# 0xC0000054/pdn-jpegxl

Measured on AMD Instinct MI355X. Metric: megapixels/sec decode (4K lossy VarDCT), higher is better.
Workload: dtype f32

## Files before the change

pdn_jpegxl_amd/build.py:

```python
import os
import subprocess
import sys

HERE = os.path.dirname(os.path.abspath(__file__))
CSRC = os.path.join(HERE, "csrc")
LIBDIR = os.path.join(HERE, "lib")
LIBNAME = "libJpegXLFileTypeIO_X64.so"
TEST_LIBNAME = "libjxlhip_selftest.so"
TEST_SOURCES = ["selftest.cc"]
SOURCES = ["kernels.hip", "entropy_kernels.hip", "tile_kernels.hip", "encode_kernels.hip", "lossless_kernels.hip", "distance_kernels.hip", "compose_kernels.hip", "patch_kernels.hip", "noise_kernels.hip", "downscale_kernels.hip", "host_parse.cc", "host_write.cc", "icc.cc", "decoder.cc", "encoder.cc"]
HEADERS = ["dev_types.h", "dev_util.h", "modular_uniform.h", "enc_types.h", "enc_dev.h", "kernels.h", "host_parse.h", "host_write.h", "icc.h", os.path.join("..", "..", "include", "jxlfiletypeio.h")]


def lib_path():
    return os.path.join(LIBDIR, LIBNAME)


def test_lib_path():
    return os.path.join(LIBDIR, TEST_LIBNAME)


def source_digest():
    import hashlib
    h = hashlib.sha256()
    for name in SOURCES + TEST_SOURCES + HEADERS:
        with open(os.path.join(CSRC, name), "rb") as f:
            h.update(name.encode() + b"\0" + f.read() + b"\0")
    return h.hexdigest()


def manifest_text(extra=None):
    if extra is None:
        extra = os.environ.get("JXLHIP_EXTRA_CFLAGS", "")
    extra = " ".join(extra.split())
    return source_digest() + ("\nextra: " + extra if extra else "") + "\n"


def manifest_path():
    return os.path.join(LIBDIR, "sources.sha256")


def _stale(out, deps):
    if not os.path.exists(out):
        return True
# ... 64 lines not shown
```

pdn_jpegxl_amd/csrc/entropy_kernels.hip:

```cpp
#include <hip/hip_runtime.h>
#include <cstdlib>
#include "dev_types.h"
#include "dev_util.h"
#include "kernels.h"

namespace jxlhip {

namespace {

__device__ const uint8_t d_order_bucket[kNumStrategies] = {0, 1, 1, 1, 2, 3, 4, 4, 5, 5, 6, 6, 1, 1, 1, 1, 1, 1, 7, 8, 8, 9, 10, 10, 11, 12, 12};
__device__ const uint8_t d_log2cx[kNumStrategies] = {0, 0, 0, 0, 1, 2, 0, 1, 0, 2, 1, 2, 0, 0, 0, 0, 0, 0, 3, 2, 3, 4, 3, 4, 5, 4, 5};
__device__ const uint8_t d_log2cy[kNumStrategies] = {0, 0, 0, 0, 1, 2, 1, 0, 2, 0, 2, 1, 0, 0, 0, 0, 0, 0, 3, 3, 2, 4, 4, 3, 5, 5, 4};
__device__ const uint8_t d_nnz_ctx[64] = {0,   0,   31,  62,  62,  93,  93,  93,  93,  123, 123, 123, 123, 152, 152, 152, 152, 152, 152, 152, 152, 180,
                                          180, 180, 180, 180, 180, 180, 180, 180, 180, 180, 180, 206, 206, 206, 206, 206, 206, 206, 206, 206, 206, 206,
                                          206, 206, 206, 206, 206, 206, 206, 206, 206, 206, 206, 206, 206, 206, 206, 206, 206, 206, 206, 206};

__device__ __forceinline__ int CeilLog2D(uint32_t x) { return x <= 1 ? 0 : 32 - __clz(x - 1); }
__device__ __forceinline__ int32_t UnpackSigned(uint32_t u) { return (int32_t)(u >> 1) ^ -(int32_t)(u & 1); }
#ifndef JXLHIP_PRIO_SERIAL
#define JXLHIP_PRIO_SERIAL 0
#endif
#if JXLHIP_PRIO_SERIAL
#define JXL_SERIAL_PRIO() __builtin_amdgcn_s_setprio(JXLHIP_PRIO_SERIAL)
#else
#define JXL_SERIAL_PRIO() ((void)0)
#endif

__device__ __forceinline__ void SetError(const DevImage& im, uint32_t bits, int who = 0, int where = 0) {
  atomicOr(im.status, bits);
  if (who) im.status[2 + who] = (uint32_t)where + 1;
}

#define JXL_LDS __attribute__((address_space(3)))
#define JXL_GLB __attribute__((address_space(1)))
template <class T> __device__ __forceinline__ JXL_GLB T* G(T* p) { return (JXL_GLB T*)p; }
typedef int __attribute__((ext_vector_type(4))) I4;
typedef unsigned __attribute__((ext_vector_type(2))) U2;
typedef unsigned __attribute__((ext_vector_type(4))) U4;

constexpr int kRingWords = 32;
constexpr int kTopUpEvery = 16;
template <int kRing, int kBatch>
struct LaneBitsT {
  const JXL_GLB uint32_t* w;
  JXL_LDS uint32_t* ring;
  uint32_t rs;
  uint32_t nwords;
  uint32_t rd, filled;
  uint64_t buf;
  int n;
  int skip;
  uint32_t pend[kBatch];
  bool has_pend;
  JXL_GLB uint32_t* lz_win;
  uint32_t lz_mask, lz_dm, lz_copy, lz_src, lz_done, slow_err;
  __device__ __forceinline__ void SetLz(uint32_t* win, uint32_t log_size, uint32_t dist_mult) {
    lz_win = (JXL_GLB uint32_t*)win; lz_mask = (1u << log_size) - 1; lz_dm = dist_mult;
  }
  __device__ __forceinline__ void Fetch(uint32_t* v) {
    static_assert(kBatch == 4 || kBatch == 8, "one or two 16-byte loads");
    if (filled + kBatch <= nwords) {
      const U4 a = *(const JXL_GLB U4*)(w + filled);
      v[0] = a.x; v[1] = a.y; v[2] = a.z; v[3] = a.w;
      if constexpr (kBatch == 8) {
        const U4 c = *(const JXL_GLB U4*)(w + filled + 4);
        v[4] = c.x; v[5] = c.y; v[6] = c.z; v[7] = c.w;
      }
    } else {
#pragma unroll
      for (int i = 0; i < kBatch; i++) v[i] = filled + i < nwords ? w[filled + i] : 0u;
    }
  }
  __device__ __forceinline__ void Stage(const uint32_t* v) {
#pragma unroll
    for (int i = 0; i < kBatch; i++) ring[__umul24((filled + i) & (kRing - 1), rs)] = v[i];
    filled += kBatch;
  }
  __device__ __forceinline__ void Batch() {
    uint32_t v[kBatch];
    Fetch(v);
    Stage(v);
  }
  __device__ __forceinline__ void TopUpSync() {
    while (filled + kBatch <= rd + kRing) Batch();
  }
  __device__ __forceinline__ void TopUp() {
    if (has_pend) { Stage(pend); has_pend = false; }
    while (filled + kBatch <= rd + kRing && filled - rd < (uint32_t)(kRing * 3 / 4)) Batch();
    if (filled + kBatch <= rd + kRing) { Fetch(pend); has_pend = true; }
  }
  __device__ __forceinline__ void Init(const uint8_t* cs, uint64_t cs_size, uint64_t bit_off, JXL_LDS uint32_t* ring_slot, uint32_t ring_stride) {
    const uintptr_t addr = (uintptr_t)cs + (bit_off >> 3);
    const uintptr_t al = addr & ~(uintptr_t)31;
    w = (const JXL_GLB uint32_t*)al;
    ring = ring_slot; rs = ring_stride;
    const uintptr_t end = ((uintptr_t)cs + cs_size + 3) & ~(uintptr_t)3;
    nwords = end > al ? (uint32_t)((end - al) >> 2) : 0u;
    rd = 0; filled = 0; buf = 0; n = 0; has_pend = false;
    lz_win = nullptr; lz_mask = 0; lz_dm = 0; lz_copy = 0; lz_src = 0; lz_done = 0; slow_err = 0;
    skip = (int)(addr - al) * 8 + (int)(bit_off & 7);
    TopUpSync();
    rd = (uint32_t)skip >> 5;
    Refill();
    const int s2 = skip & 31;
    buf >>= s2;
    n -= s2;
  }
  __device__ __forceinline__ void Refill() {
    if (n <= 32) {
      buf |= (uint64_t)ring[__umul24(rd & (kRing - 1), rs)] << n;
      n += 32;
      rd++;
    }
  }
  __device__ __forceinline__ uint32_t Read(int k) {
    Refill();
    const uint32_t v = (uint32_t)(buf & (((uint64_t)1 << k) - 1));
    buf >>= k;
    n -= k;
    return v;
  }
  __device__ uint64_t Consumed() const { return (uint64_t)rd * 32 - n - skip; }
};
typedef LaneBitsT<kRingWords, 8> LaneBits;

template <bool kLds> struct AS;
template <> struct AS<true> {
  typedef const JXL_LDS uint8_t* U8;
  typedef const JXL_LDS uint16_t* U16;
  typedef const JXL_LDS uint32_t* U32;
  typedef const JXL_LDS uint64_t* U64;
  typedef const JXL_LDS I4* Tree;
  typedef JXL_LDS int32_t* Row;
};
template <> struct AS<false> {
  typedef const uint8_t* U8;
  typedef const uint16_t* U16;
  typedef const uint32_t* U32;
  typedef const uint64_t* U64;
  typedef const I4* Tree;
  typedef int32_t* Row;
};

template <bool kLds>
struct CodeTab {
  typename AS<kLds>::U8 cmap;
  typename AS<kLds>::U32 cfg;
  typename AS<kLds>::U64 alias;
  const uint32_t* direct;
  uint32_t log_alpha;
  uint32_t slow;
  const DevCode* dc;
};

__device__ __forceinline__ DevTreeNode NodeOf(I4 v) {
  DevTreeNode n;
  n.property = v.x; n.splitval = v.y; n.a = (uint32_t)v.z; n.b = (uint32_t)v.w;
  return n;
}

template <class Bits>
__device__ __forceinline__ uint32_t HybridTail(Bits& b, uint32_t c, uint32_t sym) {
  const uint32_t se = c & 0xF, split = 1u << se;
  if (sym < split) return sym;
  const uint32_t msb = (c >> 4) & 0xF, lsb = (c >> 8) & 0xF;
  const uint32_t nb = se - (msb + lsb) + ((sym - split) >> (msb + lsb));
  const uint32_t low = sym & ((1u << lsb) - 1);
  const uint32_t t = sym >> lsb;
  const uint32_t bits = b.Read(nb > 32 ? 32 : nb);
  const uint32_t hi = (1u << msb) | (t & ((1u << msb) - 1));
  return (uint32_t)(((((uint64_t)hi << nb) | bits) << lsb) | low);
}

template <bool kLds>
__device__ __forceinline__ uint32_t AnsSym(LaneBits& b, uint32_t& state, typename AS<kLds>::U64 abase, uint32_t log_alpha) {
  const uint32_t le = 12 - log_alpha;
  const uint32_t res = state & 0xFFF, i = res >> le, pos = res & ((1u << le) - 1);
  const uint64_t e = abase[i];
  const uint32_t x = (uint32_t)e, y = (uint32_t)(e >> 32);
  const bool g = pos >= (x & 0xFF);
  const uint32_t sym = g ? ((x >> 8) & 0xFF) : i;
  const uint32_t off = g ? (y & 0xFFFF) + pos : pos;
  const uint32_t freq = g ? ((x >> 16) ^ (y >> 16)) : (x >> 16);
  state = __umul24(freq, state >> 12) + off;
  if (state < 65536u) state = (state << 16) | b.Read(16);
  return sym;
}

template <bool kLds>
__device__ __forceinline__ uint64_t AnsPrefetch(uint32_t state, typename AS<kLds>::U64 abase, uint32_t log_alpha) {
  return abase[(state & 0xFFF) >> (12 - log_alpha)];
}
template <bool kLds>
__device__ __forceinline__ uint32_t AnsSymPf(LaneBits& b, uint32_t& state, typename AS<kLds>::U64 abase, uint32_t log_alpha, uint64_t& e) {
  const uint32_t le = 12 - log_alpha;
  const uint32_t res = state & 0xFFF, i = res >> le, pos = res & ((1u << le) - 1);
  const uint32_t x = (uint32_t)e, y = (uint32_t)(e >> 32);
  const bool g = pos >= (x & 0xFF);
  const uint32_t sym = g ? ((x >> 8) & 0xFF) : i;
  const uint32_t off = g ? (y & 0xFFFF) + pos : pos;
  const uint32_t freq = g ? ((x >> 16) ^ (y >> 16)) : (x >> 16);
  state = __umul24(freq, state >> 12) + off;
  if (state < 65536u) state = (state << 16) | b.Read(16);
  e = abase[(state & 0xFFF) >> le];
  return sym;
}

__device__ const int8_t d_special_dist[120][2] = {
    {0, 1}, {1, 0}, {1, 1}, {-1, 1}, {0, 2}, {2, 0}, {1, 2}, {-1, 2}, {2, 1}, {-2, 1}, {2, 2}, {-2, 2}, {0, 3}, {3, 0}, {1, 3},
    {-1, 3}, {3, 1}, {-3, 1}, {2, 3}, {-2, 3}, {3, 2}, {-3, 2}, {0, 4}, {4, 0}, {1, 4}, {-1, 4}, {4, 1}, {-4, 1}, {3, 3}, {-3, 3},
    {2, 4}, {-2, 4}, {4, 2}, {-4, 2}, {0, 5}, {3, 4}, {-3, 4}, {4, 3}, {-4, 3}, {5, 0}, {1, 5}, {-1, 5}, {5, 1}, {-5, 1}, {2, 5},
    {-2, 5}, {5, 2}, {-5, 2}, {4, 4}, {-4, 4}, {3, 5}, {-3, 5}, {5, 3}, {-5, 3}, {0, 6}, {6, 0}, {1, 6}, {-1, 6}, {6, 1}, {-6, 1},
    {2, 6}, {-2, 6}, {6, 2}, {-6, 2}, {4, 5}, {-4, 5}, {5, 4}, {-5, 4}, {3, 6}, {-3, 6}, {6, 3}, {-6, 3}, {0, 7}, {7, 0}, {1, 7},
    {-1, 7}, {5, 5}, {-5, 5}, {7, 1}, {-7, 1}, {4, 6}, {-4, 6}, {6, 4}, {-6, 4}, {2, 7}, {-2, 7}, {7, 2}, {-7, 2}, {3, 7}, {-3, 7},
    {7, 3}, {-7, 3}, {5, 6}, {-5, 6}, {6, 5}, {-6, 5}, {8, 0}, {4, 7}, {-4, 7}, {7, 4}, {-7, 4}, {8, 1}, {8, 2}, {6, 6}, {-6, 6},
    {8, 3}, {5, 7}, {-5, 7}, {7, 5}, {-7, 5}, {8, 4}, {6, 7}, {-6, 7}, {7, 6}, {-7, 6}, {8, 5}, {7, 7}, {-7, 7}, {8, 6}, {8, 7}};

template <bool kLds, class Bits>
__device__ __forceinline__ uint32_t SlowSymbol(Bits& b, uint32_t& state, const CodeTab<kLds>& t, uint32_t cl) {
  const DevCode& dc = *t.dc;
  if (dc.slow & 1) {
    const uint32_t c = t.cfg[cl];
    if (c & 0x1000) return c >> 16;
    b.Refill();
    const uint32_t bits = (uint32_t)b.buf;
    const uint16_t* cnt = dc.pfx_count + cl * 16;
    int code = 0, first = 0, index = 0;
    for (int l = 1; l < 16; l++) {
      code |= (bits >> (l - 1)) & 1;
      const int k = cnt[l];
      if (code - k < first) {
        b.buf >>= l; b.n -= l;
        return dc.pfx_sorted[dc.pfx_off[cl] + index + code - first];
      }
      index += k; first = (first + k) << 1; code <<= 1;
    }
    b.slow_err = 1;
// ... 35 lines not shown
    dist = min(dist, min(b.lz_done, 1u << 20));
    if (dist == 0 || b.lz_done > b.lz_mask + 1) { b.slow_err = 1; return 0; }
    b.lz_src = b.lz_done - dist;
    b.lz_copy = len - 1;
    const uint32_t v = b.lz_win[(b.lz_src++) & b.lz_mask];
    b.lz_win[(b.lz_done++) & b.lz_mask] = v;
    return v;
  }
  const uint32_t v = HybridTail(b, t.cfg[cl], sym);
  if (lz) b.lz_win[(b.lz_done++) & b.lz_mask] = v;
  return v;
}
template <bool kLds, class Bits>
__device__ __forceinline__ uint32_t InitAnsState(Bits& b, const CodeTab<kLds>& t) { return (t.slow & 1) ? 0x130000u : b.Read(32); }

template <bool kLds, class Bits>
__device__ __forceinline__ uint32_t AnsGet(Bits& b, uint32_t& state, const CodeTab<kLds>& t, uint32_t ctx) {
  if (t.slow) return SlowGet(b, state, t, ctx);
  const uint32_t cl = t.cmap[ctx];
  const uint32_t le = 12 - t.log_alpha;
  const uint32_t res = state & 0xFFF, i = res >> le, pos = res & ((1u << le) - 1);
  const uint64_t e = t.alias[(cl << t.log_alpha) | i];
  const uint32_t c = t.cfg[cl];
  const uint32_t x = (uint32_t)e, y = (uint32_t)(e >> 32);
  const bool g = pos >= (x & 0xFF);
  const uint32_t sym = g ? ((x >> 8) & 0xFF) : i;
  const uint32_t off = g ? (y & 0xFFFF) + pos : pos;
  const uint32_t freq = g ? ((x >> 16) ^ (y >> 16)) : (x >> 16);
  state = __umul24(freq, state >> 12) + off;
  if (state < 65536u) state = (state << 16) | b.Read(16);
  return HybridTail(b, c, sym);
}

__device__ __forceinline__ size_t StageCode(JXL_LDS uint8_t* smem, size_t off, const DevCode& dc, CodeTab<true>& t, int tid, int nt,
                                            bool one_section = false) {
  const uint32_t na = (dc.slow & 1) ? 0u : dc.num_clusters << dc.log_alpha;
  t.direct = (one_section && !dc.slow) ? dc.direct : nullptr;
  off = (off + 7) & ~(size_t)7;
  JXL_LDS uint64_t* sa = (JXL_LDS uint64_t*)(smem + off); off += (size_t)na * 8;
  JXL_LDS uint32_t* sc = (JXL_LDS uint32_t*)(smem + off); off += (size_t)dc.num_clusters * 4;
  JXL_LDS uint8_t* sm = smem + off; off += dc.num_ctx;
  for (uint32_t i = tid; i < na; i += nt) sa[i] = dc.alias[i];
  for (uint32_t i = tid; i < dc.num_clusters; i += nt) sc[i] = dc.cfg[i];
  for (uint32_t i = tid; i < dc.num_ctx; i += nt) sm[i] = dc.ctx_map[i];
  t.cmap = sm; t.cfg = sc; t.alias = sa; t.log_alpha = dc.log_alpha; t.slow = dc.slow; t.dc = &dc;
  return off;
}

__device__ __forceinline__ void GlobalCode(const DevCode& dc, CodeTab<false>& t) {
  t.cmap = dc.ctx_map; t.cfg = dc.cfg; t.alias = dc.alias; t.direct = nullptr; t.log_alpha = dc.log_alpha; t.slow = dc.slow; t.dc = &dc;
}

template <bool kLds>
struct RowBuf {
  typename AS<kLds>::Row rb;
  int rb_stride;
  int rb_width;
};

template <bool kLds, int kPred>
__device__ __forceinline__ void LeafRow(LaneBits& b, uint32_t& state, const CodeTab<kLds>& tab, const DevTreeNode& leaf, int w, int y,
                                        JXL_GLB int32_t* row, int stride, typename AS<kLds>::Row rb, int rs, bool use_rb) {
  const uint32_t cl = tab.cmap[leaf.a >> 8];
  const uint32_t cfg = tab.cfg[cl];
  const typename AS<kLds>::U64 abase = tab.alias + (cl << tab.log_alpha);
  const bool constant_token = (cfg & 0x1000) && ((cfg >> 16) & 0xFF) < (1u << (cfg & 0xF));
  const uint32_t const_res = (uint32_t)UnpackSigned((cfg >> 16) & 0xFF) * leaf.b + (uint32_t)leaf.splitval;
  const JXL_GLB int32_t* prow = row - stride;
  int32_t W = y ? (use_rb ? rb[0] : prow[0]) : 0, N = W, NW = W;
  uint64_t entry = constant_token ? 0 : AnsPrefetch<kLds>(state, abase, tab.log_alpha);
  for (int x = 0; x < w; x++) {
    if ((x & (kTopUpEvery - 1)) == 0) b.TopUp();
    int32_t NE = N;
    if (kPred != 0 && kPred != 1) {
      if (x + 1 < w && y) NE = use_rb ? rb[(x + 1) * rs] : prow[x + 1];
    }
    uint32_t guess;
    if (kPred == 0) guess = 0;
    else if (kPred == 1) guess = (uint32_t)W;
    else if (kPred == 2) guess = (uint32_t)N;
    else {
      const int64_t mn = W < N ? W : N, mx = W < N ? N : W, gr = (int64_t)W + N - NW;
      guess = (uint32_t)(int32_t)(gr < mn ? mn : (gr > mx ? mx : gr));
    }
    uint32_t res;
    if (constant_token) res = const_res;
    else {
      const uint32_t sym = AnsSymPf<kLds>(b, state, abase, tab.log_alpha, entry);
      res = (uint32_t)UnpackSigned(HybridTail(b, cfg, sym)) * leaf.b + (uint32_t)leaf.splitval;
    }
    const int32_t val = (int32_t)(res + guess);
    row[x] = val;
    if (use_rb) rb[x * rs] = val;
    W = val;
    if (y) { NW = N; N = NE; } else { NW = val; N = val; }
  }
}

struct WpState {
  int32_t* err;
  uint32_t* pe;
  int w2;
  int64_t prediction[4];
  int64_t pred;
  __device__ void Init(int32_t* scratch, int w) {
    w2 = w + 2;
    err = scratch;
    pe = (uint32_t*)(err + 2 * w2);
    for (int i = 0; i < 10 * w2; i++) err[i] = 0;
  }
  static __device__ __forceinline__ uint32_t Div(uint32_t i) { return (1u << 24) / (i + 1); }
  static __device__ __forceinline__ uint32_t ErrorWeight(uint64_t x, uint32_t maxweight) {
    int shift = (63 - __clzll((long long)(x + 1))) - 5;
    if (shift < 0) shift = 0;
    return 4 + (uint32_t)((maxweight * (uint64_t)Div((uint32_t)(x >> shift))) >> shift);
  }
  static __device__ __forceinline__ int64_t Abs(int64_t v) { return v < 0 ? -v : v; }
  __device__ int64_t Predict(int x, int y, int w, int64_t N, int64_t W, int64_t NE, int64_t NW, int64_t NN, int64_t* max_err) {
    const int cur = (y & 1) ? 0 : w2, prev = (y & 1) ? w2 : 0;
    const int pN = prev + x, pNE = x < w - 1 ? pN + 1 : pN, pNW = x > 0 ? pN - 1 : pN;
    const uint32_t kW[4] = {13, 12, 12, 12};
    uint32_t weights[4];
// ... 327 lines not shown
    const uint32_t cl = tab.cmap[nd.a >> 8];
    const uint32_t cfg = tab.cfg[cl];
    const typename AS<kLds>::U64 abase = tab.alias + (cl << tab.log_alpha);
    const uint32_t mul = nd.b, off = (uint32_t)nd.splitval;
    const bool add_w = !needs_n && (nd.a & 0xFF) == 1;
    const uint32_t csym = (cfg >> 16) & 0xFF;
    const bool ctok = (cfg & 0x1000) && csym < (1u << (cfg & 0xF));
    const uint32_t cres = (uint32_t)UnpackSigned(csym) * mul + off;
    JXL_GLB int32_t* const row = out + (size_t)y * stride;
    uint32_t W = y ? first_prev : 0u;
    if (ctok) {
      for (int x = 0; x < w; x++) {
        const uint32_t val = cres + (add_w ? W : 0u);
        row[x] = (int32_t)val;
        W = val;
      }
      first_prev = cres + (add_w ? (y ? first_prev : 0u) : 0u);
      continue;
    }
    uint32_t first = 0;
    if constexpr (kLds) {
      if (tab.direct) {
        const uint64_t ga = (uint64_t)(uintptr_t)(tab.direct + (cl << 12));
        const ConstU32 dt = (ConstU32)(((uint64_t)(uint32_t)__builtin_amdgcn_readfirstlane((int)(ga >> 32)) << 32) |
                                       (uint32_t)__builtin_amdgcn_readfirstlane((int)(uint32_t)ga));
        if (mul == 1 && off == 0 && needs_n) RowScalar<true, ConstU32>(b, state, dt, cfg, 1u, 0u, false, W, first, row, w);
        else RowScalar<false, ConstU32>(b, state, dt, cfg, mul, off, add_w, W, first, row, w);
        first_prev = first;
        continue;
      }
    }
    uint64_t entry = AnsPrefetch<kLds>(state, abase, tab.log_alpha);
    for (int x0 = 0; x0 < w; x0 += kTopUpEvery) {
      b.TopUp();
      const int xe = min(w, x0 + kTopUpEvery);
      for (int x = x0; x < xe; x++) {
        const uint32_t sym = AnsSymPf<kLds>(b, state, abase, tab.log_alpha, entry);
        const uint32_t val = (uint32_t)UnpackSigned(HybridTail(b, cfg, sym)) * mul + off + (add_w ? W : 0u);
        row[x] = (int32_t)val;
        W = val;
        first = x == 0 ? val : first;
      }
    }
    first_prev = first;
  }
  d.kind = needs_n ? kChanResid : kChanFinal;
  *desc = d;
}

__device__ __forceinline__ int32_t FromLaneBelow(int32_t v) {
  return __builtin_amdgcn_update_dpp(0, v, 0x138 , 0xF, 0xF, false);
}
__device__ __forceinline__ int32_t ClampedGradient32(int32_t W, int32_t N, int32_t NW) {
  const int32_t mn = W < N ? W : N, mx = W < N ? N : W;
  return NW >= mx ? mn : (NW <= mn ? mx : (int32_t)((uint32_t)W + (uint32_t)N - (uint32_t)NW));
}
__device__ __forceinline__ uint32_t RowGuess(uint32_t pred, int32_t W, int32_t N, int32_t NW) {
  const uint32_t g = (uint32_t)ClampedGradient32(W, N, NW);
  return pred == 0 ? 0u : (pred == 1 ? (uint32_t)W : (pred == 2 ? (uint32_t)N : g));
}
template <bool kU8Out>
__device__ void PredictWave(const I4* tree, int chan, int sid, int32_t* plane_generic, int stride, int w, int h, int kind, int32_t cvalue,
                            uint8_t* out8_generic, int out_stride, JXL_LDS int32_t* carry, int lane) {
  JXL_GLB int32_t* const plane = G(plane_generic);
  JXL_GLB uint8_t* const out8 = G(out8_generic);
  for (int y0 = 0; y0 < h; y0 += 64) {
    const int nrows = min(64, h - y0);
    const int y = y0 + lane;
    const bool row_active = lane < nrows;
    uint32_t pred = 0;
    if (row_active) { bool u = false; pred = RowNode(tree, chan, sid, y, &u).a & 0xFF; }
// ... 569 lines not shown
    const uint64_t pf_t0 = clock64();
    pf_periods++;
#endif
    b.TopUp();
    if (dpend_n) {
#pragma unroll
      for (int i = 0; i < kQ; i++) if ((uint32_t)i < dpend_n) dq[__umul24((dfilled + i) & dqmask, nslots)] = dpend[i];
      dfilled += dpend_n;
      dpend_n = 0;
    }
    if (dfilled < min(nblk, bi + kQ)) {
      const uint32_t lim = min(nblk, bi + kQ);
      uint32_t v[kQ];
#pragma unroll
      for (int i = 0; i < kQ; i++) { v[i] = 0u; if (dfilled + i < lim) v[i] = list[dfilled + i]; }
#pragma unroll
      for (int i = 0; i < kQ; i++) if (dfilled + i < lim) dq[__umul24((dfilled + i) & dqmask, nslots)] = v[i];
      dfilled = lim;
    }
    {
      const uint32_t lim = min(nblk, bi + 2 * kQ);
      if (dfilled < lim) {
        dpend_n = min(lim - dfilled, (uint32_t)kQ);
#pragma unroll
        for (int i = 0; i < kQ; i++) { dpend[i] = 0u; if ((uint32_t)i < dpend_n) dpend[i] = list[dfilled + i]; }
      }
    }
#ifdef JXLHIP_PROFILE_HF
    pf_period += clock64() - pf_t0;
#endif
  };
  if (per_wave > 1 && !tab.slow) {
    while (!err) {
      if ((it & (kTop - 1)) == 0) period();
      auto colv = [&](uint32_t c, uint32_t x) { return (uint32_t)col[__umul24(c * 32 + x, nslots)]; };
      auto look_ahead = [&]() {
        const uint32_t x = d_next & 31, xl = x ? x - 1 : 0;
        up0 = colv(1, x); lf0 = colv(1, xl);
        up1 = colv(0, x); lf1 = colv(0, xl);
        up2 = colv(2, x); lf2 = colv(2, xl);
      };
      if (want_nz && ci >= 3) {
        if (bi >= nblk) break;
        if (bi == 0) {
          d_next = dq[0];
          d_after = dq[__umul24(1u & dqmask, nslots)];
          look_ahead();
          pcx = 0;
        }
        const uint32_t d = d_next;
        bx = d & 31; by = (d >> 5) & 31;
        lcx = (d >> 10) & 7;
        const uint32_t lcy = (d >> 13) & 7;
        ctxs = d >> 16;
        log2c = lcx + lcy; covered = 1u << log2c; size = covered << 6;
        cell = __umul24(by, w8) + bx;
        ci = 0;
        const uint32_t xl = bx ? bx - 1 : 0;
        const bool up_prev = bx - pbx < pcx, lf_prev = xl - pbx < pcx;
        auto nz_ctx = [&](uint32_t up, uint32_t lf, uint32_t fv, uint32_t block_ctx) {
          const uint32_t a = up_prev ? fv : up, l = lf_prev ? fv : lf;
          uint32_t p = bx == 0 ? (by == 0 ? 32u : a) : (by == 0 ? l : (a + l + 1) >> 1);
          p = p >= 64 ? 64 : p;
          p = p < 8 ? p : 4 + p / 2;
          return ctx_offset + p * nbc + block_ctx;
        };
        nz_ctx0 = nz_ctx(up0, lf0, fv0, ctxs & 31);
        nz_ctx1 = nz_ctx(up1, lf1, fv1, (ctxs >> 5) & 31);
        nz_ctx2 = nz_ctx(up2, lf2, fv2, (ctxs >> 10) & 31);
        pbx = bx; pcx = 1u << lcx;
        bi++;
        d_next = d_after;
        look_ahead();
        d_after = dq[__umul24((bi + 1) & dqmask, nslots)];
      }
      const uint32_t nzl = (nzeros + covered - 1) >> log2c;
      const uint32_t ks = k >> log2c;
      const uint32_t fctx = min(ks - 1, min(7 + (ks >> 1), 15 + (ks >> 2)));
      const uint32_t nzc = ci == 0 ? nz_ctx0 : (ci == 1 ? nz_ctx1 : nz_ctx2);
      const uint32_t u = AnsGet(b, state, tab, want_nz ? nzc : histo + (NnzBucketCtx(nzl) + fctx) * 2 + prev);
      it++;
      if (want_nz) {
        nzeros = u;
        if (nzeros + covered > size) { err |= kErrBitstream; break; }
        const uint32_t fill = (nzeros + covered - 1) >> log2c;
        const int c = ci == 0 ? 1 : (ci == 1 ? 0 : 2);
        JXL_LDS uint8_t* const cc = col + __umul24(c * 32 + bx, nslots);
        for (uint32_t ix = 0; ix < (1u << lcx); ix++) cc[__umul24(ix, nslots)] = (uint8_t)fill;
        fv0 = ci == 0 ? fill : fv0; fv1 = ci == 1 ? fill : fv1; fv2 = ci == 2 ? fill : fv2;
        U2 rec;
        rec.x = epos; rec.y = nzeros;
        cblk[(size_t)c * ncells + cell] = rec;
        if (nzeros) {
          const uint32_t block_ctx = (ctxs >> (5 * ci)) & 31;
          histo = ctx_offset + nbc * 37 + 458 * block_ctx;
          prev = nzeros > size / 16 ? 0 : 1;
          k = covered;
          want_nz = false;
        } else {
          ci++;
        }
      } else {
        if (u) {
          const int32_t v = UnpackSigned(u);
          if (v != (int32_t)(int16_t)v) err |= kErrRange;
          ent[epos++] = k | (uint32_t)v << 16;
          prev = 1;
          if (--nzeros == 0) { want_nz = true; ci++; }
        } else {
          prev = 0;
        }
        if (++k >= size && nzeros != 0) { err |= kErrBitstream; break; }
      }
// ... 851 lines not shown
```

pdn_jpegxl_amd/csrc/selftest.cc:

```cpp
#include <hip/hip_runtime.h>
#include <algorithm>
#include <cstring>
#include <stdexcept>
#include <string>
#include <vector>
#include "../../include/jxlfiletypeio.h"
#include "dev_util.h"
#include "enc_types.h"
#include "host_parse.h"
#include "host_write.h"
#include "icc.h"

namespace jxlhip {
std::vector<EncTreeNode> MakeEncoderTree(uint32_t nlf);
extern const int32_t kWpCutsHost[kWpLeaves - 1];
std::vector<EncTreeNode> MakeLosslessSearchTree(int nch, const int32_t* pred, bool wp_ctx, int palette, uint8_t ctx[4][kWpLeaves + 1], int* palette_ctx);
void WriteLosslessSearchHeader(BitWriter& bw, int palette_colours, int palette_channels, int rct_type);
}
using namespace jxlhip;

static void SetEncErr(ErrorInfo* e, const char* msg) {
  if (!e || !msg) return;
  size_t n = strlen(msg);
  if (n == 0) return;
  if (n > 255) n = 255;
  memcpy(e->errorMessage, msg, n);
  e->errorMessage[n] = 0;
}

namespace jxlhip {
bool ReadBackTokens(const uint8_t* bytes, size_t nbytes, size_t num_ctx, const uint32_t* ctxs, const uint32_t* values, size_t n, std::string* why);
bool ReadBackTree(const uint8_t* bytes, size_t nbytes, std::vector<DevTreeNode>* tree, std::string* why);
}

extern "C" JXLFILETYPEIO_API int32_t jxlhip_selftest_entropy(uint32_t seed, uint32_t num_ctx, uint32_t n, int32_t max_clusters,
                                                             uint32_t pinned_ctx_plus1, ErrorInfo* err) {
  try {
    uint64_t s = seed * 0x9E3779B97F4A7C15ull + 12345;
    auto rnd = [&]() { s ^= s << 13; s ^= s >> 7; s ^= s << 17; return (uint32_t)(s >> 32); };
    std::vector<uint32_t> ctxs(n), vals(n), hist((size_t)num_ctx * kEncAlphabet, 0);
// ... 79 lines not shown
    return 0;
  }
}

extern "C" JXLFILETYPEIO_API size_t jxlhip_selftest_headers_icc(uint32_t xsize, uint32_t ysize, int32_t alpha, int32_t lossless, const uint8_t* icc,
                                                                size_t icc_size, uint8_t* dst, size_t capacity) {
  try {
    EncImageInfo ii;
    ii.xsize = xsize; ii.ysize = ysize; ii.gray = false; ii.alpha = alpha != 0; ii.xyb = !lossless;
    ii.icc = icc; ii.icc_size = icc_size;
    EncFrameInfo fi;
    fi.encoding = lossless ? 1 : 0;
    fi.gab = !lossless; fi.epf_iters = lossless ? 0 : 1;
    BitWriter cs;
    WriteCodestreamHeaders(ii, cs);
    WriteFrameHeader(ii, fi, cs);
    const uint32_t ng = ((xsize + 255) / 256) * ((ysize + 255) / 256), nlf = ((xsize + 2047) / 2048) * ((ysize + 2047) / 2048);
    std::vector<uint32_t> sizes(ng == 1 ? 1 : 2 + nlf + ng, 3);
    WriteToc(sizes, cs);
    std::vector<uint8_t> bytes = cs.Finish();
    bytes.resize(bytes.size() + 3 * sizes.size(), 0);
    std::vector<uint8_t> file = WriteContainer(bytes, nullptr, 0, nullptr, 0);
    if (file.size() > capacity) return 0;
    memcpy(dst, file.data(), file.size());
    return file.size();
  } catch (...) {
    return 0;
  }
}

extern "C" JXLFILETYPEIO_API int32_t jxlhip_selftest_reflect(int32_t v, int32_t n) { return ReflectIndex(v, n); }

extern "C" JXLFILETYPEIO_API uint32_t jxlhip_selftest_nnz_ctx(uint32_t nzl) { return NnzBucketCtx(nzl); }

extern "C" JXLFILETYPEIO_API size_t jxlhip_selftest_write_tokens(uint32_t num_ctx, const uint32_t* ctxs, const uint32_t* values, uint32_t n,
                                                                 uint8_t* dst, size_t capacity, uint64_t* nbits) {
  try {
    std::vector<uint32_t> hist((size_t)num_ctx * kEncAlphabet, 0);
    std::vector<EncToken> toks;
    for (uint32_t i = 0; i < n; i++) {
      if (ctxs[i] >= num_ctx) return 0;
      uint32_t tok, nb, bits;
      HybridEncode(values[i], &tok, &nb, &bits);
      hist[(size_t)ctxs[i] * kEncAlphabet + tok]++;
      toks.push_back(EncToken{ctxs[i], values[i]});
    }
    BitWriter bw;
    EncCode code;
    BuildAndWriteCode(hist.data(), num_ctx, (int)num_ctx, std::vector<uint8_t>(num_ctx, 0), bw, code);
    WriteTokensHost(toks, code, bw);
    const uint64_t bit_count = bw.BitCount();
    std::vector<uint8_t> bytes = bw.Finish();
    if (bytes.size() > capacity) return 0;
    memcpy(dst, bytes.data(), bytes.size());
    *nbits = bit_count;
    return bytes.size();
  } catch (...) {
    return 0;
  }
}

extern "C" JXLFILETYPEIO_API int32_t jxlhip_selftest_lossless_tree(int32_t nch, const int32_t* pred, int32_t wp_ctx, int32_t palette, ErrorInfo* err) {
  try {
    uint8_t ctx[4][kWpLeaves + 1];
    int pal_ctx = -1;
    const std::vector<EncTreeNode> t = MakeLosslessSearchTree(nch, pred, wp_ctx != 0, palette, ctx, &pal_ctx);
// ... 103 lines not shown
```

Measured before the change: 31890.

## Prefetch bitstream ring words ahead and use branchless merges in ANS decode

Moves the lane bit-reader into a shared header and adds a two-word look-ahead register window (la0/la1) loaded right after each top-up or merge. ANS symbol decode, the hybrid-uint tail and state refill now use predicated merge/take operations instead of branchy Refill/Read calls. The aim is to take the dependent LDS ring reads off the serial critical path of entropy decoding and cut divergence. A sched_barrier is also added in the prefetching ANS path. The cost is extra registers and LDS reads per symbol, and it only stays correct if the look-ahead invariants hold; a host selftest for the bit window is added to check them.

```diff
diff --git a/pdn_jpegxl_amd/build.py b/pdn_jpegxl_amd/build.py
--- a/pdn_jpegxl_amd/build.py
+++ b/pdn_jpegxl_amd/build.py
@@ -9,7 +9,7 @@
 TEST_LIBNAME = "libjxlhip_selftest.so"
 TEST_SOURCES = ["selftest.cc"]
 SOURCES = ["kernels.hip", "entropy_kernels.hip", "tile_kernels.hip", "encode_kernels.hip", "lossless_kernels.hip", "distance_kernels.hip", "compose_kernels.hip", "patch_kernels.hip", "noise_kernels.hip", "downscale_kernels.hip", "host_parse.cc", "host_write.cc", "icc.cc", "decoder.cc", "encoder.cc"]
-HEADERS = ["dev_types.h", "dev_util.h", "modular_uniform.h", "enc_types.h", "enc_dev.h", "kernels.h", "host_parse.h", "host_write.h", "icc.h", os.path.join("..", "..", "include", "jxlfiletypeio.h")]
+HEADERS = ["dev_types.h", "dev_util.h", "bit_window.h", "modular_uniform.h", "enc_types.h", "enc_dev.h", "kernels.h", "host_parse.h", "host_write.h", "icc.h", os.path.join("..", "..", "include", "jxlfiletypeio.h")]
 
 
 def lib_path():
diff --git a/pdn_jpegxl_amd/csrc/bit_window.h b/pdn_jpegxl_amd/csrc/bit_window.h
--- /dev/null
+++ b/pdn_jpegxl_amd/csrc/bit_window.h
@@ -0,0 +1,131 @@
+#pragma once
+#include <stdint.h>
+
+#ifdef JXLHIP_BIT_WINDOW_HOST
+#define JXL_LDS
+#define JXL_GLB
+#define JXL_BW_FN inline
+#define JXL_BW_MUL24(a, b) ((uint32_t)(a) * (uint32_t)(b))
+#else
+#define JXL_LDS __attribute__((address_space(3)))
+#define JXL_GLB __attribute__((address_space(1)))
+#define JXL_BW_FN __device__ __forceinline__
+#define JXL_BW_MUL24(a, b) __umul24(a, b)
+#endif
+
+namespace jxlhip {
+
+constexpr int kRingWords = 32;
+constexpr int kTopUpEvery = 16;
+template <int kRing, int kBatch>
+struct LaneBitsT {
+  typedef unsigned __attribute__((ext_vector_type(4))) Quad;
+  const JXL_GLB uint32_t* w;
+  JXL_LDS uint32_t* ring;
+  uint32_t rs;
+  uint32_t nwords;
+  uint32_t rd, filled;
+  uint64_t buf;
+  int n;
+  int skip;
+  uint32_t la0, la1;
+  uint32_t pend[kBatch];
+  bool has_pend;
+  JXL_GLB uint32_t* lz_win;
+  uint32_t lz_mask, lz_dm, lz_copy, lz_src, lz_done, slow_err;
+  JXL_BW_FN void SetLz(uint32_t* win, uint32_t log_size, uint32_t dist_mult) {
+    lz_win = (JXL_GLB uint32_t*)win; lz_mask = (1u << log_size) - 1; lz_dm = dist_mult;
+  }
+  JXL_BW_FN void Fetch(uint32_t* v) {
+    static_assert(kBatch == 4 || kBatch == 8, "one or two 16-byte loads");
+    if (filled + kBatch <= nwords) {
+      const Quad a = *(const JXL_GLB Quad*)(w + filled);
+      v[0] = a.x; v[1] = a.y; v[2] = a.z; v[3] = a.w;
+      if constexpr (kBatch == 8) {
+        const Quad c = *(const JXL_GLB Quad*)(w + filled + 4);
+        v[4] = c.x; v[5] = c.y; v[6] = c.z; v[7] = c.w;
+      }
+    } else {
+#pragma unroll
+      for (int i = 0; i < kBatch; i++) v[i] = filled + i < nwords ? w[filled + i] : 0u;
+    }
+  }
+  JXL_BW_FN void Stage(const uint32_t* v) {
+#pragma unroll
+    for (int i = 0; i < kBatch; i++) ring[JXL_BW_MUL24((filled + i) & (kRing - 1), rs)] = v[i];
+    filled += kBatch;
+  }
+  JXL_BW_FN void Batch() {
+    uint32_t v[kBatch];
+    Fetch(v);
+    Stage(v);
+  }
+  JXL_BW_FN void TopUpSync() {
+    while (filled + kBatch <= rd + kRing) Batch();
+  }
+  JXL_BW_FN void TopUp() {
+    if (has_pend) { Stage(pend); has_pend = false; }
+    while (filled + kBatch <= rd + kRing && filled - rd < (uint32_t)(kRing * 3 / 4)) Batch();
+    if (filled + kBatch <= rd + kRing) { Fetch(pend); has_pend = true; }
+  }
+  JXL_BW_FN void Init(const uint8_t* cs, uint64_t cs_size, uint64_t bit_off, JXL_LDS uint32_t* ring_slot, uint32_t ring_stride) {
+    const uintptr_t addr = (uintptr_t)cs + (bit_off >> 3);
+    const uintptr_t al = addr & ~(uintptr_t)31;
+    w = (const JXL_GLB uint32_t*)al;
+    ring = ring_slot; rs = ring_stride;
+    const uintptr_t end = ((uintptr_t)cs + cs_size + 3) & ~(uintptr_t)3;
+    nwords = end > al ? (uint32_t)((end - al) >> 2) : 0u;
+    rd = 0; filled = 0; buf = 0; n = 0; has_pend = false; la0 = 0; la1 = 0;
+    lz_win = nullptr; lz_mask = 0; lz_dm = 0; lz_copy = 0; lz_src = 0; lz_done = 0; slow_err = 0;
+    skip = (int)(addr - al) * 8 + (int)(bit_off & 7);
+    TopUpSync();
+    rd = (uint32_t)skip >> 5;
+    Refill();
+    const int s2 = skip & 31;
+    buf >>= s2;
+    n -= s2;
+  }
+  JXL_BW_FN uint32_t Word(uint32_t j) const { return ring[JXL_BW_MUL24(j & (kRing - 1), rs)]; }
+  JXL_BW_FN void Refill() {
+    if (n <= 32) {
+      buf |= (uint64_t)Word(rd) << n;
+      n += 32;
+      rd++;
+    }
+  }
+  JXL_BW_FN uint32_t Read(int k) {
+    Refill();
+    const uint32_t v = (uint32_t)(buf & (((uint64_t)1 << k) - 1));
+    buf >>= k;
+    n -= k;
+    return v;
+  }
+  JXL_BW_FN void Ahead() { la0 = Word(rd); la1 = Word(rd + 1); }
+  JXL_BW_FN void TopUpAhead() { TopUp(); Ahead(); }
+  JXL_BW_FN void Merge() { MergeIf(true); }
+  JXL_BW_FN void MergeIf(bool wanted) {
+    const bool m = wanted && n <= 32;
+    const uint64_t in = (uint64_t)la0 << (n & 63);
+    buf |= m ? in : (uint64_t)0;
+    n += m ? 32 : 0;
+    rd += m ? 1u : 0u;
+    la0 = m ? la1 : la0;
+  }
+  JXL_BW_FN uint32_t Take(int k) {
+    const uint32_t v = (uint32_t)(buf & (((uint64_t)1 << k) - 1));
+    buf >>= k;
+    n -= k;
+    return v;
+  }
+  JXL_BW_FN void RefillState(uint32_t& state) {
+    const bool need = state < 65536u;
+    state = need ? (state << 16) | ((uint32_t)buf & 0xFFFFu) : state;
+    const int k = need ? 16 : 0;
+    buf >>= k;
+    n -= k;
+  }
+  JXL_BW_FN uint64_t Consumed() const { return (uint64_t)rd * 32 - n - skip; }
+};
+typedef LaneBitsT<kRingWords, 8> LaneBits;
+
+}
diff --git a/pdn_jpegxl_amd/csrc/entropy_kernels.hip b/pdn_jpegxl_amd/csrc/entropy_kernels.hip
--- a/pdn_jpegxl_amd/csrc/entropy_kernels.hip
+++ b/pdn_jpegxl_amd/csrc/entropy_kernels.hip
@@ -2,6 +2,7 @@
 #include <cstdlib>
 #include "dev_types.h"
 #include "dev_util.h"
+#include "bit_window.h"
 #include "kernels.h"
 
 namespace jxlhip {
@@ -31,98 +32,11 @@
   if (who) im.status[2 + who] = (uint32_t)where + 1;
 }
 
-#define JXL_LDS __attribute__((address_space(3)))
-#define JXL_GLB __attribute__((address_space(1)))
 template <class T> __device__ __forceinline__ JXL_GLB T* G(T* p) { return (JXL_GLB T*)p; }
 typedef int __attribute__((ext_vector_type(4))) I4;
 typedef unsigned __attribute__((ext_vector_type(2))) U2;
 typedef unsigned __attribute__((ext_vector_type(4))) U4;
 
-constexpr int kRingWords = 32;
-constexpr int kTopUpEvery = 16;
-template <int kRing, int kBatch>
-struct LaneBitsT {
-  const JXL_GLB uint32_t* w;
-  JXL_LDS uint32_t* ring;
-  uint32_t rs;
-  uint32_t nwords;
-  uint32_t rd, filled;
-  uint64_t buf;
-  int n;
-  int skip;
-  uint32_t pend[kBatch];
-  bool has_pend;
-  JXL_GLB uint32_t* lz_win;
-  uint32_t lz_mask, lz_dm, lz_copy, lz_src, lz_done, slow_err;
-  __device__ __forceinline__ void SetLz(uint32_t* win, uint32_t log_size, uint32_t dist_mult) {
-    lz_win = (JXL_GLB uint32_t*)win; lz_mask = (1u << log_size) - 1; lz_dm = dist_mult;
-  }
-  __device__ __forceinline__ void Fetch(uint32_t* v) {
-    static_assert(kBatch == 4 || kBatch == 8, "one or two 16-byte loads");
-    if (filled + kBatch <= nwords) {
-      const U4 a = *(const JXL_GLB U4*)(w + filled);
-      v[0] = a.x; v[1] = a.y; v[2] = a.z; v[3] = a.w;
-      if constexpr (kBatch == 8) {
-        const U4 c = *(const JXL_GLB U4*)(w + filled + 4);
-        v[4] = c.x; v[5] = c.y; v[6] = c.z; v[7] = c.w;
-      }
-    } else {
-#pragma unroll
-      for (int i = 0; i < kBatch; i++) v[i] = filled + i < nwords ? w[filled + i] : 0u;
-    }
-  }
-  __device__ __forceinline__ void Stage(const uint32_t* v) {
-#pragma unroll
-    for (int i = 0; i < kBatch; i++) ring[__umul24((filled + i) & (kRing - 1), rs)] = v[i];
-    filled += kBatch;
-  }
-  __device__ __forceinline__ void Batch() {
-    uint32_t v[kBatch];
-    Fetch(v);
-    Stage(v);
-  }
-  __device__ __forceinline__ void TopUpSync() {
-    while (filled + kBatch <= rd + kRing) Batch();
-  }
-  __device__ __forceinline__ void TopUp() {
-    if (has_pend) { Stage(pend); has_pend = false; }
-    while (filled + kBatch <= rd + kRing && filled - rd < (uint32_t)(kRing * 3 / 4)) Batch();
-    if (filled + kBatch <= rd + kRing) { Fetch(pend); has_pend = true; }
-  }
-  __device__ __forceinline__ void Init(const uint8_t* cs, uint64_t cs_size, uint64_t bit_off, JXL_LDS uint32_t* ring_slot, uint32_t ring_stride) {
-    const uintptr_t addr = (uintptr_t)cs + (bit_off >> 3);
-    const uintptr_t al = addr & ~(uintptr_t)31;
-    w = (const JXL_GLB uint32_t*)al;
-    ring = ring_slot; rs = ring_stride;
-    const uintptr_t end = ((uintptr_t)cs + cs_size + 3) & ~(uintptr_t)3;
-    nwords = end > al ? (uint32_t)((end - al) >> 2) : 0u;
-    rd = 0; filled = 0; buf = 0; n = 0; has_pend = false;
-    lz_win = nullptr; lz_mask = 0; lz_dm = 0; lz_copy = 0; lz_src = 0; lz_done = 0; slow_err = 0;
-    skip = (int)(addr - al) * 8 + (int)(bit_off & 7);
-    TopUpSync();
-    rd = (uint32_t)skip >> 5;
-    Refill();
-    const int s2 = skip & 31;
-    buf >>= s2;
-    n -= s2;
-  }
-  __device__ __forceinline__ void Refill() {
-    if (n <= 32) {
-      buf |= (uint64_t)ring[__umul24(rd & (kRing - 1), rs)] << n;
-      n += 32;
-      rd++;
-    }
-  }
-  __device__ __forceinline__ uint32_t Read(int k) {
-    Refill();
-    const uint32_t v = (uint32_t)(buf & (((uint64_t)1 << k) - 1));
-    buf >>= k;
-    n -= k;
-    return v;
-  }
-  __device__ uint64_t Consumed() const { return (uint64_t)rd * 32 - n - skip; }
-};
-typedef LaneBitsT<kRingWords, 8> LaneBits;
 
 template <bool kLds> struct AS;
 template <> struct AS<true> {
@@ -172,8 +86,24 @@
   return (uint32_t)(((((uint64_t)hi << nb) | bits) << lsb) | low);
 }
 
+template <class Bits>
+__device__ __forceinline__ uint32_t HybridTailAhead(Bits& b, uint32_t c, uint32_t sym) {
+  const uint32_t se = c & 0xF, split = 1u << se;
+  b.MergeIf(sym >= split);
+  b.Ahead();
+  if (sym < split) return sym;
+  const uint32_t msb = (c >> 4) & 0xF, lsb = (c >> 8) & 0xF;
+  const uint32_t nb = se - (msb + lsb) + ((sym - split) >> (msb + lsb));
+  const uint32_t low = sym & ((1u << lsb) - 1);
+  const uint32_t t = sym >> lsb;
+  const uint32_t bits = b.Take(nb > 32 ? 32 : nb);
+  const uint32_t hi = (1u << msb) | (t & ((1u << msb) - 1));
+  return (uint32_t)(((((uint64_t)hi << nb) | bits) << lsb) | low);
+}
+
 template <bool kLds>
 __device__ __forceinline__ uint32_t AnsSym(LaneBits& b, uint32_t& state, typename AS<kLds>::U64 abase, uint32_t log_alpha) {
+  b.Merge();
   const uint32_t le = 12 - log_alpha;
   const uint32_t res = state & 0xFFF, i = res >> le, pos = res & ((1u << le) - 1);
   const uint64_t e = abase[i];
@@ -183,7 +113,7 @@
   const uint32_t off = g ? (y & 0xFFFF) + pos : pos;
   const uint32_t freq = g ? ((x >> 16) ^ (y >> 16)) : (x >> 16);
   state = __umul24(freq, state >> 12) + off;
-  if (state < 65536u) state = (state << 16) | b.Read(16);
+  b.RefillState(state);
   return sym;
 }
 
@@ -193,6 +123,7 @@
 }
 template <bool kLds>
 __device__ __forceinline__ uint32_t AnsSymPf(LaneBits& b, uint32_t& state, typename AS<kLds>::U64 abase, uint32_t log_alpha, uint64_t& e) {
+  b.Merge();
   const uint32_t le = 12 - log_alpha;
   const uint32_t res = state & 0xFFF, i = res >> le, pos = res & ((1u << le) - 1);
   const uint32_t x = (uint32_t)e, y = (uint32_t)(e >> 32);
@@ -201,8 +132,9 @@
   const uint32_t off = g ? (y & 0xFFFF) + pos : pos;
   const uint32_t freq = g ? ((x >> 16) ^ (y >> 16)) : (x >> 16);
   state = __umul24(freq, state >> 12) + off;
-  if (state < 65536u) state = (state << 16) | b.Read(16);
+  b.RefillState(state);
   e = abase[(state & 0xFFF) >> le];
+  __builtin_amdgcn_sched_barrier(0);
   return sym;
 }
 
@@ -304,6 +236,24 @@
   return HybridTail(b, c, sym);
 }
 
+template <bool kLds, class Bits>
+__device__ __forceinline__ uint32_t AnsGetAhead(Bits& b, uint32_t& state, const CodeTab<kLds>& t, uint32_t ctx) {
+  b.Merge();
+  const uint32_t cl = t.cmap[ctx];
+  const uint32_t le = 12 - t.log_alpha;
+  const uint32_t res = state & 0xFFF, i = res >> le, pos = res & ((1u << le) - 1);
+  const uint64_t e = t.alias[(cl << t.log_alpha) | i];
+  const uint32_t c = t.cfg[cl];
+  const uint32_t x = (uint32_t)e, y = (uint32_t)(e >> 32);
+  const bool g = pos >= (x & 0xFF);
+  const uint32_t sym = g ? ((x >> 8) & 0xFF) : i;
+  const uint32_t off = g ? (y & 0xFFFF) + pos : pos;
+  const uint32_t freq = g ? ((x >> 16) ^ (y >> 16)) : (x >> 16);
+  state = __umul24(freq, state >> 12) + off;
+  b.RefillState(state);
+  return HybridTailAhead(b, c, sym);
+}
+
 __device__ __forceinline__ size_t StageCode(JXL_LDS uint8_t* smem, size_t off, const DevCode& dc, CodeTab<true>& t, int tid, int nt,
                                             bool one_section = false) {
   const uint32_t na = (dc.slow & 1) ? 0u : dc.num_clusters << dc.log_alpha;
@@ -342,7 +292,7 @@
   int32_t W = y ? (use_rb ? rb[0] : prow[0]) : 0, N = W, NW = W;
   uint64_t entry = constant_token ? 0 : AnsPrefetch<kLds>(state, abase, tab.log_alpha);
   for (int x = 0; x < w; x++) {
-    if ((x & (kTopUpEvery - 1)) == 0) b.TopUp();
+    if ((x & (kTopUpEvery - 1)) == 0) b.TopUpAhead();
     int32_t NE = N;
     if (kPred != 0 && kPred != 1) {
       if (x + 1 < w && y) NE = use_rb ? rb[(x + 1) * rs] : prow[x + 1];
@@ -359,7 +309,7 @@
     if (constant_token) res = const_res;
     else {
       const uint32_t sym = AnsSymPf<kLds>(b, state, abase, tab.log_alpha, entry);
-      res = (uint32_t)UnpackSigned(HybridTail(b, cfg, sym)) * leaf.b + (uint32_t)leaf.splitval;
+      res = (uint32_t)UnpackSigned(HybridTailAhead(b, cfg, sym)) * leaf.b + (uint32_t)leaf.splitval;
     }
     const int32_t val = (int32_t)(res + guess);
     row[x] = val;
@@ -753,11 +703,11 @@
     }
     uint64_t entry = AnsPrefetch<kLds>(state, abase, tab.log_alpha);
     for (int x0 = 0; x0 < w; x0 += kTopUpEvery) {
-      b.TopUp();
+      b.TopUpAhead();
       const int xe = min(w, x0 + kTopUpEvery);
       for (int x = x0; x < xe; x++) {
         const uint32_t sym = AnsSymPf<kLds>(b, state, abase, tab.log_alpha, entry);
-        const uint32_t val = (uint32_t)UnpackSigned(HybridTail(b, cfg, sym)) * mul + off + (add_w ? W : 0u);
+        const uint32_t val = (uint32_t)UnpackSigned(HybridTailAhead(b, cfg, sym)) * mul + off + (add_w ? W : 0u);
         row[x] = (int32_t)val;
         W = val;
         first = x == 0 ? val : first;
@@ -1393,7 +1343,7 @@
   };
   if (per_wave > 1 && !tab.slow) {
     while (!err) {
-      if ((it & (kTop - 1)) == 0) period();
+      if ((it & (kTop - 1)) == 0) { period(); b.Ahead(); }
       auto colv = [&](uint32_t c, uint32_t x) { return (uint32_t)col[__umul24(c * 32 + x, nslots)]; };
       auto look_ahead = [&]() {
         const uint32_t x = d_next & 31, xl = x ? x - 1 : 0;
@@ -1439,7 +1389,7 @@
       const uint32_t ks = k >> log2c;
       const uint32_t fctx = min(ks - 1, min(7 + (ks >> 1), 15 + (ks >> 2)));
       const uint32_t nzc = ci == 0 ? nz_ctx0 : (ci == 1 ? nz_ctx1 : nz_ctx2);
-      const uint32_t u = AnsGet(b, state, tab, want_nz ? nzc : histo + (NnzBucketCtx(nzl) + fctx) * 2 + prev);
+      const uint32_t u = AnsGetAhead(b, state, tab, want_nz ? nzc : histo + (NnzBucketCtx(nzl) + fctx) * 2 + prev);
       it++;
       if (want_nz) {
         nzeros = u;
diff --git a/pdn_jpegxl_amd/csrc/selftest.cc b/pdn_jpegxl_amd/csrc/selftest.cc
--- a/pdn_jpegxl_amd/csrc/selftest.cc
+++ b/pdn_jpegxl_amd/csrc/selftest.cc
@@ -6,6 +6,8 @@
 #include <vector>
 #include "../../include/jxlfiletypeio.h"
 #include "dev_util.h"
+#define JXLHIP_BIT_WINDOW_HOST
+#include "bit_window.h"
 #include "enc_types.h"
 #include "host_parse.h"
 #include "host_write.h"
@@ -151,6 +153,60 @@
 extern "C" JXLFILETYPEIO_API int32_t jxlhip_selftest_reflect(int32_t v, int32_t n) { return ReflectIndex(v, n); }
 
 extern "C" JXLFILETYPEIO_API uint32_t jxlhip_selftest_nnz_ctx(uint32_t nzl) { return NnzBucketCtx(nzl); }
+
+template <int kRing>
+static int32_t RunBitWindow(int look_ahead, const uint8_t* bytes, size_t nbytes, uint64_t bit_off, const uint8_t* widths, uint32_t ntokens,
+                            uint32_t* values, uint64_t* consumed) {
+  std::vector<uint8_t> store(nbytes + 96, 0xA5);
+  uint8_t* cs = (uint8_t*)(((uintptr_t)store.data() + 31) & ~(uintptr_t)31);
+  if (nbytes) memcpy(cs, bytes, nbytes);
+  memset(cs + nbytes, 0, 3);
+  constexpr uint32_t kStride = 3;
+  std::vector<uint32_t> ring((size_t)kRing * kStride, 0xDEADBEEFu);
+  LaneBitsT<kRing, kRing / 4> b;
+  b.Init(cs, nbytes, bit_off, ring.data() + 1, kStride);
+  for (uint32_t t = 0; t < ntokens; t++) {
+    const int k0 = widths[2 * t], k1 = widths[2 * t + 1];
+    if (k0 > 16 || k1 > 32) return -1;
+    uint32_t v0, v1;
+    if (look_ahead) {
+      if (t % (kRing / 2) == 0) b.TopUpAhead();
+      b.Merge();
+      if (k0 == 16) {
+        uint32_t state = 1;
+        b.RefillState(state);
+        v0 = state & 0xFFFFu;
+        if ((state >> 16) != 1) return -1;
+      } else {
+        uint32_t state = 0x10000u;
+        b.RefillState(state);
+        if (state != 0x10000u) return -1;
+        v0 = b.Take(k0);
+      }
+      consumed[2 * t] = b.Consumed();
+      b.MergeIf(k1 != 0);
+      b.Ahead();
+      v1 = b.Take(k1);
+      consumed[2 * t + 1] = b.Consumed();
+    } else {
+      if (t % (kRing / 2) == 0) b.TopUp();
+      v0 = b.Read(k0);
+      consumed[2 * t] = b.Consumed();
+      v1 = b.Read(k1);
+      consumed[2 * t + 1] = b.Consumed();
+    }
+    values[2 * t] = v0;
+    values[2 * t + 1] = v1;
+  }
+  return 0;
+}
+extern "C" JXLFILETYPEIO_API int32_t jxlhip_selftest_bit_window(int32_t ring_words, int32_t look_ahead, const uint8_t* bytes, size_t nbytes,
+                                                                uint64_t bit_off, const uint8_t* widths, uint32_t ntokens, uint32_t* values,
+                                                                uint64_t* consumed) {
+  if (ring_words == 32) return RunBitWindow<32>(look_ahead, bytes, nbytes, bit_off, widths, ntokens, values, consumed);
+  if (ring_words == 16) return RunBitWindow<16>(look_ahead, bytes, nbytes, bit_off, widths, ntokens, values, consumed);
+  return -1;
+}
 
 extern "C" JXLFILETYPEIO_API size_t jxlhip_selftest_write_tokens(uint32_t num_ctx, const uint32_t* ctxs, const uint32_t* values, uint32_t n,
                                                                  uint8_t* dst, size_t capacity, uint64_t* nbits) {
```

Measured after the change: 28850. 0.905x the previous value.
